# robo-alex/gs-dynamics

Measured on AMD Instinct MI355X. Metric: fwd+bwd Mpix/s at 100k Gaussians, 4x800^2 views, higher is better.
Workload: dtype f32

## Files before the change

### gs-dynamics_amd/csrc/gsr_binning.hip

```cpp
#include "gsr_common.h"

namespace gsr_binning {

#define SCAN_THREADS 1024
#define SCAN_ITEMS 8
__global__ __launch_bounds__(SCAN_THREADS) void scan_exclusive_kernel(const uint32_t* __restrict__ in,
                                                                      uint32_t* __restrict__ out, uint32_t n,
                                                                      uint32_t* __restrict__ total_out) {
  __shared__ uint32_t wave_tot[SCAN_THREADS / GSR_WAVE];
  __shared__ uint32_t carry_s;
  const int tid = threadIdx.x, lane = tid & 63, wv = tid >> 6;
  if (tid == 0) carry_s = 0;
  __syncthreads();
  const uint32_t per_round = SCAN_THREADS * SCAN_ITEMS;
  for (uint32_t base = 0; base < n; base += per_round) {
    uint32_t v[SCAN_ITEMS];
    uint32_t first = base + (uint32_t)tid * SCAN_ITEMS;
    uint32_t sum = 0;
#pragma unroll
    for (int k = 0; k < SCAN_ITEMS; ++k) {
      uint32_t idx = first + k;
      v[k] = idx < n ? in[idx] : 0u;
      sum += v[k];
    }
// ... 616 lines not shown
  const int Ts = gsr_bin_stride(tab.T), rows = tab.rows, t = blockIdx.x * GSR_BLOCK + threadIdx.x;
  if (t >= Ts) return;
  uint32_t* __restrict__ m = vw.tile_rows;
  uint32_t run = 0;
  int r = 0;
  for (; r + 8 <= rows; r += 8) {
    uint32_t v[8];
#pragma unroll
    for (int u = 0; u < 8; ++u) v[u] = m[(size_t)(r + u) * Ts + t];
#pragma unroll
    for (int u = 0; u < 8; ++u) { m[(size_t)(r + u) * Ts + t] = run; run += v[u]; }
  }
  for (; r < rows; ++r) { const uint32_t v = m[(size_t)r * Ts + t]; m[(size_t)r * Ts + t] = run; run += v; }
  m[(size_t)rows * Ts + t] = run;
}

__global__ __launch_bounds__(GSR_BLOCK) void bin_colprefix_scan_kernel(GsrBinViews tab) {
  const GsrBinView& vw = tab.v[blockIdx.y];
  if (vw.shares_lists) return;
  __shared__ uint32_t s_w[GSR_BLOCK / 64];
  __shared__ uint32_t s_base;
  const int T = tab.T, Ts = gsr_bin_stride(T), rows = tab.rows, tid = threadIdx.x, lane = tid & 63, wv = tid >> 6;
  const int t = blockIdx.x * GSR_BLOCK + tid;
  uint32_t* __restrict__ m = vw.tile_rows;
  uint32_t run = 0;
  if (t < Ts) {
    int r = 0;
    for (; r + 8 <= rows; r += 8) {
      uint32_t v[8];
#pragma unroll
      for (int u = 0; u < 8; ++u) v[u] = m[(size_t)(r + u) * Ts + t];
#pragma unroll
      for (int u = 0; u < 8; ++u) { m[(size_t)(r + u) * Ts + t] = run; run += v[u]; }
    }
    for (; r < rows; ++r) { const uint32_t v = m[(size_t)r * Ts + t]; m[(size_t)r * Ts + t] = run; run += v; }
    m[(size_t)rows * Ts + t] = run;
  }
  uint32_t inc = run;
#pragma unroll
  for (int d = 1; d < 64; d <<= 1) {
    const uint32_t o = __shfl_up(inc, d, 64);
    if (lane >= d) inc += o;
  }
  if (lane == 63) s_w[wv] = inc;
  __syncthreads();
  uint32_t before = 0, total = 0;
#pragma unroll
  for (int w = 0; w < GSR_BLOCK / 64; ++w) { if (w < wv) before += s_w[w]; total += s_w[w]; }
  uint32_t* __restrict__ words = vw.block_hist;
  if (tid == 0) __hip_atomic_store(&words[blockIdx.x], 0x80000000u | total, __ATOMIC_RELAXED, __HIP_MEMORY_SCOPE_AGENT);
  if (wv == 0) {
    uint32_t mine = 0;
    if (lane < (int)blockIdx.x) {
      uint32_t w;
      do { w = __hip_atomic_load(&words[lane], __ATOMIC_RELAXED, __HIP_MEMORY_SCOPE_AGENT); } while (!(w & 0x80000000u));
      mine = w & 0x7fffffffu;
    }
#pragma unroll
    for (int k = 32; k >= 1; k >>= 1) mine += __shfl_xor(mine, k, 64);
    if (lane == 0) s_base = mine;
  }
  __syncthreads();
  const uint32_t start = s_base + before + inc - run, cap = vw.D;
  if (t < T) vw.ranges[t] = make_uint2(min(start, cap), min(start + run, cap));
}

__device__ __forceinline__ void bin_scan_view(const GsrBinViews& tab, const GsrBinView& vw, int prefixed, uint32_t* s_wave, uint32_t* s_carry) {
  const int T = tab.T, Ts = gsr_bin_stride(T), rows = tab.rows, tid = threadIdx.x, lane = tid & 63, wv = tid >> 6;
  uint32_t* __restrict__ m = vw.tile_rows;
  const uint32_t cap = vw.D;
  if (tid == 0) *s_carry = 0;
  __syncthreads();
  for (int q0 = 0; q0 < Ts / 4; q0 += BIN_THREADS) {
    const int q = q0 + tid;
    const bool live = q < Ts / 4;
    uint4 tot = make_uint4(0u, 0u, 0u, 0u);
    if (live) {
      if (prefixed) tot = *reinterpret_cast<const uint4*>(m + (size_t)rows * Ts + 4 * q);
      else {
        for (int r0 = 0; r0 < rows; r0 += BIN_ROW_CHUNK) {
          uint4 v[BIN_ROW_CHUNK];
#pragma unroll
          for (int r = 0; r < BIN_ROW_CHUNK; ++r)
            v[r] = r0 + r < rows ? *reinterpret_cast<const uint4*>(m + (size_t)(r0 + r) * Ts + 4 * q) : make_uint4(0u, 0u, 0u, 0u);
#pragma unroll
          for (int r = 0; r < BIN_ROW_CHUNK; ++r)
            if (r0 + r < rows) {
              *reinterpret_cast<uint4*>(m + (size_t)(r0 + r) * Ts + 4 * q) = tot;
              tot.x += v[r].x; tot.y += v[r].y; tot.z += v[r].z; tot.w += v[r].w;
            }
        }
      }
    }
    const uint32_t mine = tot.x + tot.y + tot.z + tot.w;
    uint32_t inc = mine;
#pragma unroll
    for (int d = 1; d < 64; d <<= 1) {
      const uint32_t o = __shfl_up(inc, d, 64);
      if (lane >= d) inc += o;
    }
    if (lane == 63) s_wave[wv] = inc;
    __syncthreads();
    uint32_t start = *s_carry + inc - mine;
    for (int w = 0; w < wv; ++w) start += s_wave[w];
    if (live) {
      const uint32_t c[4] = {tot.x, tot.y, tot.z, tot.w};
      uint32_t st_ = start;
#pragma unroll
      for (int k = 0; k < 4; ++k) {
        if (4 * q + k < T) vw.ranges[4 * q + k] = make_uint2(min(st_, cap), min(st_ + c[k], cap));
        st_ += c[k];
      }
    }
    __syncthreads();
    if (tid == BIN_THREADS - 1) *s_carry = start + mine;
    __syncthreads();
  }
}

__global__ __launch_bounds__(BIN_THREADS) void bin_scan_kernel(GsrBinViews tab, int prefixed) {
  __shared__ uint32_t s_wave[BIN_THREADS / 64];
  __shared__ uint32_t s_carry;
  const GsrBinView& vw = tab.v[blockIdx.x];
  if (vw.shares_lists) return;
  bin_scan_view(tab, vw, prefixed, s_wave, &s_carry);
}

__global__ __launch_bounds__(BIN_THREADS) void bin_emit_kernel(int P, GsrBinViews tab, int order_wgs, int items_per_wg) {
  extern __shared__ uint32_t s_cur[];
  if ((int)blockIdx.x >= tab.rows) {
    __shared__ TileOrderLds L;
    if (blockIdx.y == 0) tile_order_body(tab, items_per_wg, (int)blockIdx.x - tab.rows, L);
    return;
  }
  (void)order_wgs;
  __shared__ uint2 s_big[BIN_BIG_MAX];
  __shared__ uint64_t s_bigkey[BIN_BIG_MAX];
  __shared__ uint32_t s_nbig;
  const GsrBinView& vw = tab.v[blockIdx.y];
  const int T = tab.T, Ts = gsr_bin_stride(T), gx = tab.gx, tid = threadIdx.x, lane = tid & 63, wv = tid >> 6;
  const int g0 = (int)blockIdx.x * GSR_BIN_G;
  if (vw.shares_lists) return;
  const uint32_t cap = vw.D;
  const uint32_t* __restrict__ row = vw.tile_rows + (size_t)blockIdx.x * Ts;
  const uint32_t* __restrict__ cut = vw.depth_cut;
  const bool cut_l = cut && tab.cut_lds;
  const uint32_t* s_cut = s_cur + T;
  const uint32_t* s_cc = s_cur + 2 * T;
  const int gxc = (gx + 3) >> 2;
  if (cut_l)
    for (int t = tid; t < T; t += BIN_THREADS) s_cur[T + t] = cut[t];
  auto cut_at = [&](uint32_t t) { return cut_l ? s_cut[t] : cut[t]; };
  auto behind_all = [&](uint2 r, uint32_t dbits) {
    const uint32_t x0 = (r.x & 0xffffu) >> 2, y0 = (r.x >> 16) >> 2, x1 = ((r.y & 0xffffu) - 1u) >> 2, y1 = ((r.y >> 16) - 1u) >> 2;
    uint32_t m = 0u;
    for (uint32_t y = y0; y <= y1; ++y)
      for (uint32_t x = x0; x <= x1; ++x) m = max(m, s_cc[y * gxc + x]);
    return dbits > m;
  };
  uint64_t* __restrict__ dg = vw.dg[0];
  uint2 rc[BIN_PER_THREAD], ek[BIN_PER_THREAD];
#pragma unroll
  for (int q = 0; q < BIN_PER_THREAD; ++q) {
    const int g = g0 + tid * BIN_PER_THREAD + q;
    rc[q] = make_uint2(0u, 0u); ek[q] = rc[q];
    if (g < P) { rc[q] = vw.rect[g]; ek[q] = vw.ekey[g]; }
  }
  if (tid == 0) s_nbig = 0;
  for (int t = tid; t < T; t += BIN_THREADS) s_cur[t] = vw.ranges[t].x + row[t];
  __syncthreads();
  if (cut_l) {
    const int gyc = (T / gx + 3) >> 2;
    for (int c = tid; c < gxc * gyc; c += BIN_THREADS) {
      const int cx = c % gxc, cy = c / gxc;
      uint32_t m = 0u;
      for (int y = 4 * cy; y < min(4 * cy + 4, T / gx); ++y)
        for (int x = 4 * cx; x < min(4 * cx + 4, gx); ++x) m = max(m, s_cut[y * gx + x]);
      s_cur[2 * T + c] = m;
    }
    __syncthreads();
  }
#pragma unroll
  for (int q = 0; q < BIN_PER_THREAD; ++q) {
    const BinGauss b = bin_gauss(rc[q], ek[q].y);
    if (b.area == 0u) continue;
    if (cut_l && behind_all(rc[q], ek[q].x)) continue;
    const uint64_t key = ((uint64_t)ek[q].x << 32) | (uint32_t)(g0 + tid * BIN_PER_THREAD + q);
    if (b.area > BIN_BIG_AREA) {
      const uint32_t slot = atomicAdd(&s_nbig, 1u);
      if (slot < BIN_BIG_MAX) { s_big[slot] = rc[q]; s_bigkey[slot] = key; continue; }
    }
    const uint32_t dbits = ek[q].x;
    bin_for_tiles(b, gx, [&](uint32_t t) {
      if (cut && dbits > cut_at(t)) return;
      const uint32_t slot = atomicAdd(&s_cur[t], 1u);
      if (slot < cap) dg[slot] = key;
    });
  }
  __syncthreads();
  const uint32_t nbig = min(s_nbig, (uint32_t)BIN_BIG_MAX);
  for (uint32_t i = wv; i < nbig; i += BIN_THREADS / 64) {
    const BinGauss b = bin_gauss(s_big[i], 0u);
    const uint64_t key = s_bigkey[i];
    for (uint32_t k = lane; k < b.area; k += 64) {
      const uint32_t t = bin_tile_of(b, k, gx);
      if (cut && (uint32_t)(key >> 32) > cut_at(t)) continue;
      const uint32_t slot = atomicAdd(&s_cur[t], 1u);
      if (slot < cap) dg[slot] = key;
    }
  }
}

__global__ __launch_bounds__(GSR_BLOCK) void tile_ranges_kernel(GsrBinViews tab, int cur) {
  const GsrBinView& vw = tab.v[blockIdx.y];
  const uint32_t* __restrict__ tkey = vw.tkey[cur];
  uint2* __restrict__ ranges = vw.ranges;
  const uint32_t D = bin_entries(vw);
  uint32_t i = blockIdx.x * GSR_BLOCK + threadIdx.x;
  if (i >= D) return;
  uint32_t t = tkey[i];
  if (i == 0) ranges[t].x = 0;
  else {
    uint32_t pt = tkey[i - 1];
    if (pt != t) { ranges[pt].y = i; ranges[t].x = i; }
  }
  if (i == D - 1) ranges[t].y = D;
}


template <typename PTR>
__device__ __forceinline__ void tile_sort_network(PTR a, uint32_t n, int tid, const uint32_t NT = GSR_BLOCK) {
  uint32_t lg = 1;
  while ((1u << lg) < n) ++lg;
  const uint32_t npairs = (1u << lg) >> 1;
  for (uint32_t lk = 1; lk <= lg; ++lk) {
    const uint32_t k = 1u << lk, hk = k >> 1;
    for (uint32_t p = tid; p < npairs; p += NT) {
      const uint32_t base = (p >> (lk - 1)) << lk, off = p & (hk - 1);
      const uint32_t l = base + off, r = base + (k - 1 - off);
      if (r < n) {
        uint64_t x = a[l], y = a[r];
        if (y < x) { a[l] = y; a[r] = x; }
      }
    }
    __syncthreads();
    for (int lj = (int)lk - 2; lj >= 0; --lj) {
      const uint32_t j = 1u << lj;
      for (uint32_t p = tid; p < npairs; p += NT) {
        const uint32_t l = ((p >> lj) << (lj + 1)) + (p & (j - 1)), r = l + j;
        if (r < n) {
          uint64_t x = a[l], y = a[r];
          if (y < x) { a[l] = y; a[r] = x; }
        }
      }
      __syncthreads();
    }
  }
}

template <int M>
__device__ __forceinline__ uint32_t gsr_lane_xor(uint32_t v) {
  if constexpr (M == 1) return (uint32_t)__builtin_amdgcn_update_dpp(0, (int)v, 0xB1, 0xf, 0xf, true);
  else if constexpr (M == 2) return (uint32_t)__builtin_amdgcn_update_dpp(0, (int)v, 0x4E, 0xf, 0xf, true);
  else if constexpr (M == 3) return (uint32_t)__builtin_amdgcn_update_dpp(0, (int)v, 0x1B, 0xf, 0xf, true);
  else if constexpr (M == 7) return (uint32_t)__builtin_amdgcn_update_dpp(0, (int)v, 0x141, 0xf, 0xf, true);
  else if constexpr (M == 15) return (uint32_t)__builtin_amdgcn_update_dpp(0, (int)v, 0x140, 0xf, 0xf, true);
  else if constexpr (M == 8) return (uint32_t)__builtin_amdgcn_update_dpp(0, (int)v, 0x128, 0xf, 0xf, true);
  else if constexpr (M < 32) return (uint32_t)__builtin_amdgcn_ds_swizzle((int)v, (M << 10) | 0x1F);
  else return (uint32_t)__shfl_xor((int)v, M, 64);
}
template <int V> struct gsr_log2 { static constexpr int value = 1 + gsr_log2<(V >> 1)>::value; };
template <> struct gsr_log2<1> { static constexpr int value = 0; };
template <int MASK, int NR>
__device__ __forceinline__ void wave_sort_step(uint64_t (&x)[NR], int lane) {
  constexpr int LR = gsr_log2<NR>::value;
  constexpr int R = MASK & (NR - 1), L = MASK >> LR;
  constexpr int HB = MASK >= 1024 ? 1024 : MASK >= 512 ? 512 : MASK >= 256 ? 256 : MASK >= 128 ? 128 : MASK >= 64 ? 64 : MASK >= 32 ? 32 : MASK >= 16 ? 16 : MASK >= 8 ? 8 : MASK >= 4 ? 4 : MASK >= 2 ? 2 : 1;
  if constexpr (L == 0) {
#pragma unroll
    for (int r = 0; r < NR; ++r) {
      if ((r & HB) == 0) {
        const uint64_t a = x[r], b = x[r ^ R];
        const bool sw = b < a;
        x[r] = sw ? b : a;
        x[r ^ R] = sw ? a : b;
      }
    }
  } else {
    uint64_t y[NR];
#pragma unroll
    for (int r = 0; r < NR; ++r) {
      const uint64_t src = x[r ^ R];
      y[r] = ((uint64_t)gsr_lane_xor<L>((uint32_t)(src >> 32)) << 32) | gsr_lane_xor<L>((uint32_t)src);
    }
    const bool upper = (lane & (HB >> LR)) != 0;
#pragma unroll
    for (int r = 0; r < NR; ++r) {
      const bool take = (y[r] < x[r]) != upper;
      x[r] = take ? y[r] : x[r];
    }
  }
}
template <int LK, int NR>
__device__ __forceinline__ void wave_sort_stage(uint64_t (&x)[NR], int lane) {
  static_assert(LK <= 11, "the half-cleaner steps below stop at stride 512");
  wave_sort_step<(1 << LK) - 1, NR>(x, lane);
  if constexpr (LK >= 11) wave_sort_step<512, NR>(x, lane);
  if constexpr (LK >= 10) wave_sort_step<256, NR>(x, lane);
  if constexpr (LK >= 9) wave_sort_step<128, NR>(x, lane);
  if constexpr (LK >= 8) wave_sort_step<64, NR>(x, lane);
  if constexpr (LK >= 7) wave_sort_step<32, NR>(x, lane);
  if constexpr (LK >= 6) wave_sort_step<16, NR>(x, lane);
  if constexpr (LK >= 5) wave_sort_step<8, NR>(x, lane);
  if constexpr (LK >= 4) wave_sort_step<4, NR>(x, lane);
  if constexpr (LK >= 3) wave_sort_step<2, NR>(x, lane);
  if constexpr (LK >= 2) wave_sort_step<1, NR>(x, lane);
}
template <int NR>
__device__ __forceinline__ void wave_sort_tile(const uint64_t* __restrict__ seg, uint32_t* __restrict__ out, uint32_t n, int lane) {
  uint64_t x[NR];
#pragma unroll
  for (int r = 0; r < NR; ++r) { const uint32_t e = (uint32_t)(r * 64 + lane); x[r] = e < n ? seg[e] : ~0ull; }
  wave_sort_stage<1, NR>(x, lane); wave_sort_stage<2, NR>(x, lane); wave_sort_stage<3, NR>(x, lane);
  wave_sort_stage<4, NR>(x, lane); wave_sort_stage<5, NR>(x, lane); wave_sort_stage<6, NR>(x, lane);
  if constexpr (NR >= 2) wave_sort_stage<7, NR>(x, lane);
  if constexpr (NR >= 4) wave_sort_stage<8, NR>(x, lane);
  if constexpr (NR >= 8) wave_sort_stage<9, NR>(x, lane);
  if constexpr (NR >= 16) wave_sort_stage<10, NR>(x, lane);
  if constexpr (NR >= 32) wave_sort_stage<11, NR>(x, lane);
  const uint32_t e0 = (uint32_t)lane * NR;
  if constexpr (NR >= 4) {
    if ((((uintptr_t)out) & 15u) == 0 && e0 + NR <= n) {
#pragma unroll
      for (int r = 0; r < NR; r += 4)
        *reinterpret_cast<uint4*>(out + e0 + r) = make_uint4((uint32_t)x[r], (uint32_t)x[r + 1], (uint32_t)x[r + 2], (uint32_t)x[r + 3]);
      return;
    }
  }
#pragma unroll
  for (int r = 0; r < NR; ++r) if (e0 + r < n) out[e0 + r] = (uint32_t)x[r];
}

template <int RCAP, int NW = 4>
struct TileSortLds {
  union {
    struct { uint32_t key[2][RCAP]; uint32_t val[2][RCAP]; } r;
    uint64_t net[2 * RCAP];
  };
  uint32_t whist[NW][256];
  uint32_t wtot[4];
  uint32_t diff;
};

template <int RCAP, int NW>
__device__ __forceinline__ int tile_radix_sort(TileSortLds<RCAP, NW>& L, uint32_t n, int tid) {
  constexpr int NT = 64 * NW;
  const int lane = tid & 63, wv = tid >> 6;
  const uint32_t q = ((n + (uint32_t)NT - 1u) / (uint32_t)NT) << 6;
  const uint32_t wstart = min(n, (uint32_t)wv * q), wstop = min(n, wstart + q);
  const uint32_t diff = L.diff;
  int cur = 0;
  for (int shift = 0; shift < 32; shift += 8) {
    if (((diff >> shift) & 0xffu) == 0u) continue;
    const uint32_t* __restrict__ kin = L.r.key[cur];
    const uint32_t* __restrict__ vin = L.r.val[cur];
    uint32_t* __restrict__ kout = L.r.key[cur ^ 1];
    uint32_t* __restrict__ vout = L.r.val[cur ^ 1];
    for (int i = tid; i < NW * 256; i += NT) (&L.whist[0][0])[i] = 0;
    __syncthreads();
    for (uint32_t i = wstart + lane; i < wstop; i += 64) atomicAdd(&L.whist[wv][(kin[i] >> shift) & 0xffu], 1u);
    __syncthreads();
    {
      uint32_t c[NW], tot = 0;
      if (tid < 256) {
#pragma unroll
        for (int w = 0; w < NW; ++w) { c[w] = L.whist[w][tid]; tot += c[w]; }
      }
      uint32_t inc = tot;
#pragma unroll
      for (int d = 1; d < 64; d <<= 1) {
        const uint32_t o = __shfl_up(inc, d, 64);
        if (lane >= d) inc += o;
      }
      if (tid < 256 && lane == 63) L.wtot[wv] = inc;
      __syncthreads();
      if (tid < 256) {
        uint32_t base = inc - tot;
        for (int w = 0; w < wv; ++w) base += L.wtot[w];
#pragma unroll
        for (int w = 0; w < NW; ++w) { L.whist[w][tid] = base; base += c[w]; }
      }
    }
    __syncthreads();
    volatile uint32_t* wbase = L.whist[wv];
    for (uint32_t i0 = wstart; i0 < wstop; i0 += 64) {
      const uint32_t i = i0 + lane;
      const bool valid = i < wstop;
      uint32_t key = 0, val = 0;
      if (valid) { key = kin[i]; val = vin[i]; }
      const uint32_t digit = (key >> shift) & 0xffu;
      const uint64_t peers = match_peers(digit, valid, 8);
      const uint32_t rank = (uint32_t)__popcll(peers & gsr_lanemask_lt());
      uint32_t pos = 0;
      if (valid) pos = wbase[digit] + rank;
      __builtin_amdgcn_wave_barrier();
      if (valid && rank == 0) wbase[digit] = pos + (uint32_t)__popcll(peers);
      __builtin_amdgcn_wave_barrier();
      if (valid) { kout[pos] = key; vout[pos] = val; }
    }
    __syncthreads();
    cur ^= 1;
  }
  return cur;
}

template <int RCAP, int NW>
__device__ __forceinline__ void tile_sort_long_ticket(const GsrBinViews& tab, int cur, uint32_t ticket);

#ifndef TS_W32_WAVES
#define TS_W32_WAVES 5
#endif
#ifndef TS_MIN_WAVES
#define TS_MIN_WAVES 7
#endif
template <int RCAP, int MODE = 0, int NW = 4>
__global__ __launch_bounds__(64 * NW, (RCAP <= 1024 || MODE == 2) ? TS_MIN_WAVES : (MODE == 3 ? TS_W32_WAVES : 1)) void tile_sort_kernel(GsrBinViews tab, int cur) {
  const int tid = threadIdx.x;
  if constexpr (MODE == 3) {
    const uint32_t n_long3 = tab.queue[6], n_mid = tab.queue[3];
    const uint32_t ticket = n_long3 + blockIdx.x * 4u + (uint32_t)(tid >> 6);
    if (ticket >= n_mid) return;
    const uint4 ord = tab.order[ticket];
    const GsrBinView& vw = tab.v[__builtin_amdgcn_readfirstlane(ord.w)];
    if (vw.shares_lists) return;
    const uint32_t n = __builtin_amdgcn_readfirstlane(ord.z - ord.y);
    wave_sort_tile<32>(vw.dg[cur] + ord.y, vw.point_list + ord.y, n, tid & 63);
    return;
  }
  const uint32_t n_busy = tab.queue[4], n_long = tab.queue[6];
  if (MODE == 2 || (MODE == 0 && blockIdx.x >= n_long)) {
    const uint32_t first = (MODE == 2 && tab.wave_cap == 2048) ? tab.queue[3] : n_long;
    const uint32_t ticket = first + (MODE == 2 ? blockIdx.x : blockIdx.x - n_long) * 4u + (uint32_t)(tid >> 6);
    if (ticket >= n_busy) return;
    const uint4 ord = tab.order[ticket];
    const GsrBinView& vw = tab.v[__builtin_amdgcn_readfirstlane(ord.w)];
    if (vw.shares_lists) return;
    const uint32_t n = __builtin_amdgcn_readfirstlane(ord.z - ord.y);
    const uint64_t* seg = vw.dg[cur] + ord.y;
    uint32_t* out = vw.point_list + ord.y;
    if (n <= 64) wave_sort_tile<1>(seg, out, n, tid & 63);
    else if (n <= 128) wave_sort_tile<2>(seg, out, n, tid & 63);
    else if (n <= 256) wave_sort_tile<4>(seg, out, n, tid & 63);
    else if (n <= 512) wave_sort_tile<8>(seg, out, n, tid & 63);
    else wave_sort_tile<16>(seg, out, n, tid & 63);
    return;
  }
  if constexpr (MODE == 1) {
    const uint32_t n_mine = tab.wave_cap == 512 ? tab.queue[2] : n_long;
    for (uint32_t ticket = blockIdx.x; ticket < n_mine; ticket += gridDim.x) {
      tile_sort_long_ticket<RCAP, NW>(tab, cur, ticket);
      __syncthreads();
    }
  } else if constexpr (MODE != 2) {
    if (blockIdx.x >= n_long) return;
    if (RCAP <= 1024 && tab.vlong_launch && blockIdx.x < tab.queue[2]) return;
    tile_sort_long_ticket<RCAP, NW>(tab, cur, blockIdx.x);
  }
}

template <int RCAP, int NW>
__device__ __forceinline__ void tile_sort_long_ticket(const GsrBinViews& tab, int cur, uint32_t ticket) {
  __shared__ TileSortLds<RCAP, NW> L;
  constexpr uint32_t NT = 64 * NW;
  const int tid = threadIdx.x;
  const uint4 ord = tab.order[ticket];
  const GsrBinView& vw = tab.v[__builtin_amdgcn_readfirstlane(ord.w)];
  if (vw.shares_lists) return;
  uint64_t* __restrict__ dg = vw.dg[cur];
  uint32_t* __restrict__ point_list = vw.point_list;
  const uint2 rg = make_uint2(ord.y, ord.z);
  const uint32_t n = rg.y - rg.x;
  if (n == 0) return;
  uint64_t* seg = dg + rg.x;
  if (n == 1) {
    if (tid == 0) point_list[rg.x] = (uint32_t)seg[0];
  } else if (n <= (uint32_t)RCAP) {
    if (tid == 0) L.diff = 0;
    __syncthreads();
    const uint32_t k0 = (uint32_t)(seg[0] >> 32);
    uint32_t d = 0;
    for (uint32_t i = tid; i < n; i += NT) {
      const uint64_t e = seg[i];
      const uint32_t k = (uint32_t)(e >> 32);
      L.r.key[0][i] = k; L.r.val[0][i] = (uint32_t)e;
      d |= k ^ k0;
    }
    if (d) atomicOr(&L.diff, d);
    __syncthreads();
    const int cur = tile_radix_sort(L, n, tid);
    {
      uint32_t* __restrict__ kk = L.r.key[cur];
      uint32_t* __restrict__ vv = L.r.val[cur];
      bool long_run = false;
      for (uint32_t i = tid; i + 1 < n; i += NT) {
        if (kk[i] == kk[i + 1] && (i == 0 || kk[i - 1] != kk[i])) {
          uint32_t j = i + 1;
          while (j + 1 < n && kk[j + 1] == kk[i] && j - i < 32u) ++j;
          if (j + 1 < n && kk[j + 1] == kk[i]) { long_run = true; continue; }
          for (uint32_t a = i + 1; a <= j; ++a) {
            const uint32_t x = vv[a];
            uint32_t b = a;
            while (b > i && vv[b - 1] > x) { vv[b] = vv[b - 1]; --b; }
            vv[b] = x;
          }
        }
      }
      if (__syncthreads_or(long_run ? 1 : 0)) {
        uint64_t e[(RCAP + NT - 1) / NT];
#pragma unroll
        for (int u = 0; u < (RCAP + NT - 1) / NT; ++u) {
          const uint32_t i = (uint32_t)u * NT + tid;
          e[u] = i < n ? (((uint64_t)kk[i] << 32) | vv[i]) : 0ull;
        }
        __syncthreads();
#pragma unroll
        for (int u = 0; u < (RCAP + NT - 1) / NT; ++u) {
          const uint32_t i = (uint32_t)u * NT + tid;
          if (i < n) L.net[i] = e[u];
        }
        __syncthreads();
        tile_sort_network(L.net, n, tid, NT);
        for (uint32_t i = tid; i < n; i += NT) point_list[rg.x + i] = (uint32_t)L.net[i];
        return;
      }
    }
    for (uint32_t i = tid; i < n; i += NT) point_list[rg.x + i] = L.r.val[cur][i];
  } else if (n <= 2u * (uint32_t)RCAP) {
    for (uint32_t i = tid; i < n; i += NT) L.net[i] = seg[i];
    __syncthreads();
    tile_sort_network(L.net, n, tid, NT);
    for (uint32_t i = tid; i < n; i += NT) point_list[rg.x + i] = (uint32_t)L.net[i];
  } else {
    __syncthreads();
    tile_sort_network((volatile uint64_t*)seg, n, tid, NT);
    for (uint32_t i = tid; i < n; i += NT) point_list[rg.x + i] = (uint32_t)seg[i];
  }
}

__global__ __launch_bounds__(GSR_BLOCK) void copy_tile_state_kernel(int T, int n_order, const uint2* __restrict__ src_ranges,
                                                                    const uint4* __restrict__ src_order, const uint32_t* __restrict__ src_queue,
                                                                    uint2* __restrict__ ranges, uint4* __restrict__ order, uint32_t* __restrict__ queue) {
  const int i = blockIdx.x * GSR_BLOCK + threadIdx.x;
  if (i < T) ranges[i] = src_ranges[i];
  if (i < n_order) order[i] = src_order[i];
  if (i < 9) queue[i] = (i == 4 || i == 6 || i == 7) ? src_queue[i] : 0u;
}

}
using namespace gsr_binning;

int gsr_launch_shared_lists(const GsrBinViews& tab_in, int P, uint32_t D, const uint2* owner_ranges, const uint4* owner_order,
                            const uint32_t* owner_queue, uint2* ranges, uint4* order, uint32_t* queue, hipStream_t st) {
  GsrBinViews tab = tab_in;
  tab.v[0].shares_lists = 1;
  { GSR_PROF("emit_entries", st);
    hipLaunchKernelGGL(emit_entries_kernel, dim3(D / GSR_RADIX_EPB + 1u, 1), dim3(GSR_BLOCK), 0, st, P, tab, 0, 1); }
  GSR_HIP_CHECK(hipGetLastError());
  { GSR_PROF("copy_tile_state", st);
    hipLaunchKernelGGL(copy_tile_state_kernel, dim3((tab.T + GSR_BLOCK - 1) / GSR_BLOCK), dim3(GSR_BLOCK), 0, st, tab.T, tab.T, owner_ranges,
                       owner_order, owner_queue, ranges, order, queue); }
  GSR_HIP_CHECK(hipGetLastError());
  return 0;
}

int gsr_launch_scan_exclusive(const uint32_t* in, uint32_t* out, uint32_t n, uint32_t* total_out, hipStream_t st) {
  { GSR_PROF("scan", st);
  hipLaunchKernelGGL(scan_exclusive_kernel, dim3(1), dim3(SCAN_THREADS), 0, st, in, out, n, total_out); }
  GSR_HIP_CHECK(hipGetLastError());
  return 0;
}

static int ceil_log2_u32(uint32_t n) {
  int b = 0;
  while (((uint64_t)1 << b) < n) ++b;
  return b;
}

static size_t bin_lds_limit() {
  static const size_t v = [] {
    int dev = 0, a = 0;
    if (hipGetDevice(&dev) == hipSuccess && hipDeviceGetAttribute(&a, hipDeviceAttributeMaxSharedMemoryPerBlock, dev) == hipSuccess && a > 0) return (size_t)a;
    return (size_t)(64 << 10);
  }();
  return v;
}
static size_t bin_lds_static() {
  static const size_t v = [] {
    hipFuncAttributes a{}, b{};
    size_t m = 0;
    if (hipFuncGetAttributes(&a, reinterpret_cast<const void*>(bin_emit_kernel)) == hipSuccess) m = a.sharedSizeBytes;
    if (hipFuncGetAttributes(&b, reinterpret_cast<const void*>(bin_count_kernel)) == hipSuccess && b.sharedSizeBytes > m) m = b.sharedSizeBytes;
    return m ? m : (size_t)(52 << 10);
  }();
  return v;
}
bool gsr_rows_path_ok(int T) {
  const char* e = getenv("GSR_RADIX_BINNING");
  const bool radix_only = e && *e && atoi(e) != 0;
  return !radix_only && T > 0 && T <= GSR_BIN_MAX_T && bin_lds_static() + sizeof(uint32_t) * (size_t)T <= bin_lds_limit();
}
int gsr_launch_binning(const GsrBinViews& tab_in, int P, hipStream_t st) {
  if (tab_in.V <= 0 || tab_in.T <= 0) return 0;
  GsrBinViews tab = tab_in;
  uint32_t maxD = 0, maxblk = 0;
  for (int v = 0; v < tab.V; ++v) { maxD = tab.v[v].D > maxD ? tab.v[v].D : maxD; maxblk = tab.v[v].nblocks > maxblk ? tab.v[v].nblocks : maxblk; }
  const char* force = getenv("GSR_TILE_SORT_RCAP");
  const bool big = force ? (force[0] == '4') : (maxD / (uint32_t)tab.T > 600u);
  tab.wave_cap = big ? 2048 : 512;
  {
    static uint32_t* hint = [] { uint32_t* p = nullptr; if (hipHostMalloc((void**)&p, 64, hipHostMallocMapped | hipHostMallocCoherent) != hipSuccess) return (uint32_t*)nullptr; *p = 1u; return p; }();
    tab.vlong_out = hint;
    tab.vlong_launch = (!hint || __atomic_load_n(hint, __ATOMIC_RELAXED) != 0u) ? 1 : 0;
  }
  int cur = 0;
  bool order_done = false;
  bool any_cut = false;
  for (int v = 0; v < tab.V; ++v) any_cut = any_cut || tab.v[v].depth_cut != nullptr;
  const size_t coarse = (size_t)((tab.gx + 3) / 4) * (size_t)((tab.T / tab.gx + 3) / 4);
  tab.cut_lds = (any_cut && bin_lds_static() + sizeof(uint32_t) * (2 * (size_t)tab.T + coarse) <= bin_lds_limit()) ? 1 : 0;
  const size_t lds = sizeof(uint32_t) * (tab.cut_lds ? 2 * (size_t)tab.T + coarse : (size_t)tab.T);
  const bool rows_path = tab.rows > 0 && gsr_rows_path_ok(tab.T) && maxD > 0 && P > 0;
  if (rows_path) {
    { GSR_PROF("bin_count", st);
      hipLaunchKernelGGL(bin_count_kernel, dim3(tab.rows, tab.V), dim3(BIN_THREADS), lds, st, P, tab);
    }
    GSR_HIP_CHECK(hipGetLastError());
    const int prefixed = tab.rows > BIN_DIRECT_ROWS ? 1 : 0;
    const int col_wgs = (gsr_bin_stride(tab.T) + GSR_BLOCK - 1) / GSR_BLOCK;
    const bool chained = prefixed && col_wgs <= 64;
    if (chained) {
      GSR_PROF("bin_colprefix", st);
      hipLaunchKernelGGL(bin_colprefix_scan_kernel, dim3(col_wgs, tab.V), dim3(GSR_BLOCK), 0, st, tab);
    } else if (prefixed) {
      GSR_PROF("bin_colprefix", st);
      hipLaunchKernelGGL(bin_colprefix_kernel, dim3(col_wgs, tab.V), dim3(GSR_BLOCK), 0, st, tab);
    }
    GSR_HIP_CHECK(hipGetLastError());
    const int n_items = tab.V * ((tab.T + 1023) / 1024);
    if (!chained) {
      GSR_PROF("bin_scan", st);
      hipLaunchKernelGGL(bin_scan_kernel, dim3(tab.V), dim3(BIN_THREADS), 0, st, tab, prefixed);
    }
    GSR_HIP_CHECK(hipGetLastError());
    int order_wgs = 0, per_wg = 1;
    {
      order_wgs = n_items < ORD_MAX_WG ? n_items : ORD_MAX_WG;
      if (order_wgs < 1) order_wgs = 1;
      per_wg = (n_items + order_wgs - 1) / order_wgs;
      if (per_wg < 1) per_wg = 1;
      order_wgs = (n_items + per_wg - 1) / per_wg;
      if (order_wgs < 1) order_wgs = 1;
      order_done = true;
    }
    { GSR_PROF("bin_emit", st);
      hipLaunchKernelGGL(bin_emit_kernel, dim3(tab.rows + order_wgs, tab.V), dim3(BIN_THREADS), lds, st, P, tab, order_wgs, per_wg); }
    GSR_HIP_CHECK(hipGetLastError());
  } else if (maxD == 0 || P <= 0) {
    for (int v = 0; v < tab.V; ++v) GSR_HIP_CHECK(hipMemsetAsync(tab.v[v].ranges, 0, sizeof(uint2) * (size_t)tab.T, st));
  } else {
    const int tbits = ceil_log2_u32((uint32_t)tab.T);
    const int npass = (tbits + 7) / 8;
    const int bpp = npass ? (tbits + npass - 1) / npass : 0;
    { GSR_PROF("emit_entries", st);
    const int bits0 = npass ? (tbits < bpp ? tbits : bpp) : 1;
    hipLaunchKernelGGL(emit_entries_kernel, dim3(maxD / GSR_RADIX_EPB + 1u, tab.V), dim3(GSR_BLOCK), 0, st, P, tab, 0, bits0); }
    GSR_HIP_CHECK(hipGetLastError());
    for (int pass = 0; pass < npass; ++pass) {
      const int shift = pass * bpp;
      const int bits = (tbits - shift) < bpp ? (tbits - shift) : bpp;
      if (pass > 0) {
        GSR_PROF("radix_hist", st);
        hipLaunchKernelGGL(radix_hist_kernel, dim3(maxblk, tab.V), dim3(GSR_BLOCK), 0, st, tab, cur, shift, bits);
      }
      GSR_HIP_CHECK(hipGetLastError());
      const int prescanned = maxblk >= GSR_COLSCAN_MIN_BLOCKS ? 1 : 0;
      if (prescanned) {
        GSR_PROF("radix_colscan", st);
        hipLaunchKernelGGL(radix_colscan_kernel, dim3(1u << bits, tab.V), dim3(1024), 0, st, tab, bits);
      }
      GSR_HIP_CHECK(hipGetLastError());
      { GSR_PROF("radix_scatter", st);
      hipLaunchKernelGGL(radix_scatter_kernel, dim3(maxblk, tab.V), dim3(GSR_BLOCK), 0, st, tab, cur, shift, bits, prescanned,
                         pass == npass - 1 ? 1 : 0); }
      GSR_HIP_CHECK(hipGetLastError());
      cur ^= 1;
    }
    if (npass == 0) {
      GSR_PROF("tile_ranges", st);
      hipLaunchKernelGGL(tile_ranges_kernel, dim3((maxD + GSR_BLOCK - 1) / GSR_BLOCK, tab.V), dim3(GSR_BLOCK), 0, st, tab, cur);
    }
    GSR_HIP_CHECK(hipGetLastError());
  }
  if (!order_done)
    if (int rc = gsr_launch_tile_order(tab, st)) return rc;
  if (maxD > 0 && P > 0) {
    { GSR_PROF("tile_sort", st);
    if (big) {
      hipLaunchKernelGGL((tile_sort_kernel<2048, 2>), dim3((tab.V * tab.T + 3) / 4), dim3(GSR_BLOCK), 0, st, tab, cur);
      if (tab.wave_cap == 2048) hipLaunchKernelGGL((tile_sort_kernel<2048, 3>), dim3((tab.V * tab.T + 3) / 4), dim3(GSR_BLOCK), 0, st, tab, cur);
      const int g1 = tab.V * tab.T < 512 ? tab.V * tab.T : 512;
      hipLaunchKernelGGL((tile_sort_kernel<4096, 1, 8>), dim3(g1), dim3(512), 0, st, tab, cur);
    } else
      {
        const bool small_lds = !(force && force[0] == '2');
        if (small_lds) {
          hipLaunchKernelGGL(tile_sort_kernel<1024>, dim3(tab.V * tab.T), dim3(GSR_BLOCK), 0, st, tab, cur);
          if (tab.vlong_launch) hipLaunchKernelGGL((tile_sort_kernel<4096, 1, 16>), dim3(64), dim3(1024), 0, st, tab, cur);
        } else hipLaunchKernelGGL(tile_sort_kernel<2048>, dim3(tab.V * tab.T), dim3(GSR_BLOCK), 0, st, tab, cur);
      } }
    GSR_HIP_CHECK(hipGetLastError());
  }
  return 0;
}

int gsr_launch_tile_order(const GsrBinViews& tab, hipStream_t st) {
  { GSR_PROF("tile_order", st);
    const int n_items = tab.V * ((tab.T + 1023) / 1024);
    int wgs = n_items < ORD_MAX_WG ? n_items : ORD_MAX_WG;
    if (wgs < 1) wgs = 1;
    const int per_wg = (n_items + wgs - 1) / wgs;
    wgs = per_wg > 0 ? (n_items + per_wg - 1) / per_wg : 1;
    hipLaunchKernelGGL(tile_order_kernel, dim3(wgs < 1 ? 1 : wgs), dim3(1024), 0, st, tab, per_wg > 0 ? per_wg : 1); }
  GSR_HIP_CHECK(hipGetLastError());
  return 0;
}
```

Baseline: 5581.

## Sort long tiles with paired-wave bitonic merge through LDS instead of block radix sort

For long tiles (beyond 512 keys, when wave_cap is 512), two waves now each sort one half of the tile in registers with a bitonic network. They exchange halves through shared memory and finish with a merge and half-cleaner stages. Each 4-wave block handles two such tickets, replacing the block-wide multi-pass radix sort per long tile, and the wave-sort block indexing is shifted to make room. It also adds optional, compile-time-disabled timing trace instrumentation. The cost is more LDS traffic and added code complexity.

Measured after the change: 5725 (median of 6 runs). 2.6% higher.

```diff
diff --git a/gs-dynamics_amd/csrc/gsr_binning.hip b/gs-dynamics_amd/csrc/gsr_binning.hip
--- a/gs-dynamics_amd/csrc/gsr_binning.hip
+++ b/gs-dynamics_amd/csrc/gsr_binning.hip
@@ -942,9 +942,15 @@
   }
 }
 template <int LK, int NR>
+__device__ __forceinline__ void wave_sort_halfcleaners(uint64_t (&x)[NR], int lane);
+template <int LK, int NR>
 __device__ __forceinline__ void wave_sort_stage(uint64_t (&x)[NR], int lane) {
+  wave_sort_step<(1 << LK) - 1, NR>(x, lane);
+  wave_sort_halfcleaners<LK, NR>(x, lane);
+}
+template <int LK, int NR>
+__device__ __forceinline__ void wave_sort_halfcleaners(uint64_t (&x)[NR], int lane) {
   static_assert(LK <= 11, "the half-cleaner steps below stop at stride 512");
-  wave_sort_step<(1 << LK) - 1, NR>(x, lane);
   if constexpr (LK >= 11) wave_sort_step<512, NR>(x, lane);
   if constexpr (LK >= 10) wave_sort_step<256, NR>(x, lane);
   if constexpr (LK >= 9) wave_sort_step<128, NR>(x, lane);
@@ -957,6 +963,8 @@
   if constexpr (LK >= 2) wave_sort_step<1, NR>(x, lane);
 }
 template <int NR>
+__device__ __forceinline__ void wave_sort_store(const uint64_t (&x)[NR], uint32_t* __restrict__ out, uint32_t e0, uint32_t n);
+template <int NR>
 __device__ __forceinline__ void wave_sort_tile(const uint64_t* __restrict__ seg, uint32_t* __restrict__ out, uint32_t n, int lane) {
   uint64_t x[NR];
 #pragma unroll
@@ -968,7 +976,10 @@
   if constexpr (NR >= 8) wave_sort_stage<9, NR>(x, lane);
   if constexpr (NR >= 16) wave_sort_stage<10, NR>(x, lane);
   if constexpr (NR >= 32) wave_sort_stage<11, NR>(x, lane);
-  const uint32_t e0 = (uint32_t)lane * NR;
+  wave_sort_store<NR>(x, out, (uint32_t)lane * NR, n);
+}
+template <int NR>
+__device__ __forceinline__ void wave_sort_store(const uint64_t (&x)[NR], uint32_t* __restrict__ out, uint32_t e0, uint32_t n) {
   if constexpr (NR >= 4) {
     if ((((uintptr_t)out) & 15u) == 0 && e0 + NR <= n) {
 #pragma unroll
@@ -1055,6 +1066,91 @@
 }
 
 template <int RCAP, int NW>
+__device__ __forceinline__ TileSortLds<RCAP, NW>& tile_sort_lds() {
+  __shared__ TileSortLds<RCAP, NW> L;
+  return L;
+}
+__device__ __forceinline__ uint32_t pair_slot(uint32_t pos, uint32_t lnr) { return ((pos & ((1u << lnr) - 1u)) << 6) + (pos >> lnr); }
+template <int NR>
+__device__ __forceinline__ void pair_upper_sort(uint64_t (&x)[8], uint64_t* __restrict__ mine, const uint64_t* __restrict__ seg, uint32_t n, int lane) {
+  constexpr int LNR = gsr_log2<NR>::value;
+  uint64_t y[NR];
+#pragma unroll
+  for (int r = 0; r < NR; ++r) { const uint32_t e = 512u + (uint32_t)(r * 64 + lane); y[r] = e < n ? seg[e] : ~0ull; }
+  wave_sort_stage<1, NR>(y, lane); wave_sort_stage<2, NR>(y, lane); wave_sort_stage<3, NR>(y, lane);
+  wave_sort_stage<4, NR>(y, lane); wave_sort_stage<5, NR>(y, lane); wave_sort_stage<6, NR>(y, lane);
+  if constexpr (NR >= 2) wave_sort_stage<7, NR>(y, lane);
+  if constexpr (NR >= 4) wave_sort_stage<8, NR>(y, lane);
+  if constexpr (NR >= 8) wave_sort_stage<9, NR>(y, lane);
+#pragma unroll
+  for (int r = 0; r < NR; ++r) { mine[pair_slot((uint32_t)(lane * NR + r), LNR)] = y[r]; x[r] = y[r]; }
+}
+template <int NR>
+__device__ __forceinline__ void pair_upper_merge(uint64_t (&x)[8], const uint64_t* __restrict__ lower, uint32_t* __restrict__ out, uint32_t n, int lane) {
+  uint64_t y[NR];
+#pragma unroll
+  for (int r = 0; r < NR; ++r) {
+    const uint64_t o = lower[pair_slot(511u - (uint32_t)(lane * NR + r), 3)];
+    y[r] = o > x[r] ? o : x[r];
+  }
+  wave_sort_halfcleaners<gsr_log2<NR>::value + 7, NR>(y, lane);
+  wave_sort_store<NR>(y, out, 512u + (uint32_t)lane * NR, n);
+}
+template <int RCAP, int NW>
+__device__ __forceinline__ void tile_sort_pair_tickets(const GsrBinViews& tab, int cur, uint32_t ticket0, uint32_t n_long) {
+  static_assert(NW == 4 && 2 * RCAP >= 4 * 512, "two pairs of waves, 512 keys per wave in the network block");
+  TileSortLds<RCAP, NW>& L = tile_sort_lds<RCAP, NW>();
+  const int tid = threadIdx.x, lane = tid & 63, wv = tid >> 6;
+  const bool upper = (wv & 1) != 0;
+  const uint32_t ticket = ticket0 + (uint32_t)(wv >> 1);
+  bool live = ticket < n_long;
+  uint32_t n = 0;
+  const uint64_t* seg = nullptr;
+  uint32_t* out = nullptr;
+  if (live) {
+    const uint4 ord = tab.order[ticket];
+    const GsrBinView& vw = tab.v[__builtin_amdgcn_readfirstlane(ord.w)];
+    live = !vw.shares_lists;
+    n = __builtin_amdgcn_readfirstlane(ord.z - ord.y);
+    seg = vw.dg[cur] + ord.y;
+    out = vw.point_list + ord.y;
+  }
+  const uint32_t m = n > 512u ? n - 512u : 0u;
+  const uint32_t lnru = m <= 64u ? 0u : m <= 128u ? 1u : m <= 256u ? 2u : 3u;
+  uint64_t x[8];
+  uint64_t* mine = L.net + wv * 512;
+  if (live && !upper) {
+#pragma unroll
+    for (int r = 0; r < 8; ++r) { const uint32_t e = (uint32_t)(r * 64 + lane); x[r] = e < n ? seg[e] : ~0ull; }
+    wave_sort_stage<1, 8>(x, lane); wave_sort_stage<2, 8>(x, lane); wave_sort_stage<3, 8>(x, lane);
+    wave_sort_stage<4, 8>(x, lane); wave_sort_stage<5, 8>(x, lane); wave_sort_stage<6, 8>(x, lane);
+    wave_sort_stage<7, 8>(x, lane); wave_sort_stage<8, 8>(x, lane); wave_sort_stage<9, 8>(x, lane);
+#pragma unroll
+    for (int r = 0; r < 8; ++r) mine[pair_slot((uint32_t)(lane * 8 + r), 3)] = x[r];
+  } else if (live) {
+    if (lnru == 0u) pair_upper_sort<1>(x, mine, seg, n, lane);
+    else if (lnru == 1u) pair_upper_sort<2>(x, mine, seg, n, lane);
+    else if (lnru == 2u) pair_upper_sort<4>(x, mine, seg, n, lane);
+    else pair_upper_sort<8>(x, mine, seg, n, lane);
+  }
+  __syncthreads();
+  if (!live) return;
+  const uint64_t* theirs = L.net + (wv ^ 1) * 512;
+  if (!upper) {
+#pragma unroll
+    for (int r = 0; r < 8; ++r) {
+      const uint32_t j = 511u - (uint32_t)(lane * 8 + r);
+      if (j < (64u << lnru)) { const uint64_t o = theirs[pair_slot(j, lnru)]; x[r] = o < x[r] ? o : x[r]; }
+    }
+    wave_sort_halfcleaners<10, 8>(x, lane);
+    wave_sort_store<8>(x, out, (uint32_t)lane * 8u, n);
+  } else if (lnru == 0u) pair_upper_merge<1>(x, theirs, out, n, lane);
+  else if (lnru == 1u) pair_upper_merge<2>(x, theirs, out, n, lane);
+  else if (lnru == 2u) pair_upper_merge<4>(x, theirs, out, n, lane);
+  else pair_upper_merge<8>(x, theirs, out, n, lane);
+}
+
+template <int RCAP, int NW>
 __device__ __forceinline__ void tile_sort_long_ticket(const GsrBinViews& tab, int cur, uint32_t ticket);
 
 #ifndef TS_W32_WAVES
@@ -1063,9 +1159,23 @@
 #ifndef TS_MIN_WAVES
 #define TS_MIN_WAVES 7
 #endif
+#ifdef GSR_TRACE_SORT
+#define GSR_SORT_TRACE_MAX 65536
+__device__ uint4 g_sort_trace[GSR_SORT_TRACE_MAX];
+__device__ uint32_t g_sort_wg_start[GSR_SORT_TRACE_MAX];
+#define GSR_SORT_TRACE(ticket, kind, n)                                                                     \
+  do { if ((threadIdx.x & ((kind) == 2 ? 127 : 63)) == 0 && ((kind) != 1 || threadIdx.x == 0) && (ticket) < GSR_SORT_TRACE_MAX) \
+         g_sort_trace[ticket] = make_uint4((uint32_t)tr0, (uint32_t)wall_clock64(), blockIdx.x | ((uint32_t)(kind) << 24), n); } while (0)
+#else
+#define GSR_SORT_TRACE(ticket, kind, n) do { } while (0)
+#endif
 template <int RCAP, int MODE = 0, int NW = 4>
 __global__ __launch_bounds__(64 * NW, (RCAP <= 1024 || MODE == 2) ? TS_MIN_WAVES : (MODE == 3 ? TS_W32_WAVES : 1)) void tile_sort_kernel(GsrBinViews tab, int cur) {
   const int tid = threadIdx.x;
+#ifdef GSR_TRACE_SORT
+  unsigned long long tr0 = wall_clock64();
+  if (MODE == 0 && tid == 0 && blockIdx.x < GSR_SORT_TRACE_MAX) g_sort_wg_start[blockIdx.x] = (uint32_t)tr0;
+#endif
   if constexpr (MODE == 3) {
     const uint32_t n_long3 = tab.queue[6], n_mid = tab.queue[3];
     const uint32_t ticket = n_long3 + blockIdx.x * 4u + (uint32_t)(tid >> 6);
@@ -1075,12 +1185,29 @@
     if (vw.shares_lists) return;
     const uint32_t n = __builtin_amdgcn_readfirstlane(ord.z - ord.y);
     wave_sort_tile<32>(vw.dg[cur] + ord.y, vw.point_list + ord.y, n, tid & 63);
+    GSR_SORT_TRACE(ticket, 3, n);
     return;
   }
   const uint32_t n_busy = tab.queue[4], n_long = tab.queue[6];
-  if (MODE == 2 || (MODE == 0 && blockIdx.x >= n_long)) {
+  uint32_t wave_block0 = n_long;
+  if constexpr (MODE == 0 && RCAP <= 1024) {
+    if (tab.wave_cap == 512) {
+      const uint32_t n_vlong = min(tab.queue[2], n_long);
+      wave_block0 = n_vlong + ((n_long - n_vlong + 1u) >> 1);
+      if (blockIdx.x >= n_vlong && blockIdx.x < wave_block0) {
+        const uint32_t ticket0 = n_vlong + 2u * (blockIdx.x - n_vlong);
+        tile_sort_pair_tickets<RCAP, NW>(tab, cur, ticket0, n_long);
+#ifdef GSR_TRACE_SORT
+        const uint32_t tk = ticket0 + (uint32_t)(tid >> 7);
+        if (tk < n_long) GSR_SORT_TRACE(tk, 2, tab.order[tk].z - tab.order[tk].y);
+#endif
+        return;
+      }
+    }
+  }
+  if (MODE == 2 || (MODE == 0 && blockIdx.x >= wave_block0)) {
     const uint32_t first = (MODE == 2 && tab.wave_cap == 2048) ? tab.queue[3] : n_long;
-    const uint32_t ticket = first + (MODE == 2 ? blockIdx.x : blockIdx.x - n_long) * 4u + (uint32_t)(tid >> 6);
+    const uint32_t ticket = first + (MODE == 2 ? blockIdx.x : blockIdx.x - wave_block0) * 4u + (uint32_t)(tid >> 6);
     if (ticket >= n_busy) return;
     const uint4 ord = tab.order[ticket];
     const GsrBinView& vw = tab.v[__builtin_amdgcn_readfirstlane(ord.w)];
@@ -1093,24 +1220,30 @@
     else if (n <= 256) wave_sort_tile<4>(seg, out, n, tid & 63);
     else if (n <= 512) wave_sort_tile<8>(seg, out, n, tid & 63);
     else wave_sort_tile<16>(seg, out, n, tid & 63);
+    GSR_SORT_TRACE(ticket, 0, n);
     return;
   }
   if constexpr (MODE == 1) {
     const uint32_t n_mine = tab.wave_cap == 512 ? tab.queue[2] : n_long;
     for (uint32_t ticket = blockIdx.x; ticket < n_mine; ticket += gridDim.x) {
       tile_sort_long_ticket<RCAP, NW>(tab, cur, ticket);
+      GSR_SORT_TRACE(ticket, 1, tab.order[ticket].z - tab.order[ticket].y);
       __syncthreads();
+#ifdef GSR_TRACE_SORT
+      tr0 = wall_clock64();
+#endif
     }
   } else if constexpr (MODE != 2) {
     if (blockIdx.x >= n_long) return;
     if (RCAP <= 1024 && tab.vlong_launch && blockIdx.x < tab.queue[2]) return;
     tile_sort_long_ticket<RCAP, NW>(tab, cur, blockIdx.x);
+    GSR_SORT_TRACE(blockIdx.x, 1, tab.order[blockIdx.x].z - tab.order[blockIdx.x].y);
   }
 }
 
 template <int RCAP, int NW>
 __device__ __forceinline__ void tile_sort_long_ticket(const GsrBinViews& tab, int cur, uint32_t ticket) {
-  __shared__ TileSortLds<RCAP, NW> L;
+  TileSortLds<RCAP, NW>& L = tile_sort_lds<RCAP, NW>();
   constexpr uint32_t NT = 64 * NW;
   const int tid = threadIdx.x;
   const uint4 ord = tab.order[ticket];
@@ -1212,6 +1345,16 @@
   GSR_HIP_CHECK(hipGetLastError());
   return 0;
 }
+
+#ifdef GSR_TRACE_SORT
+extern "C" int gsr_debug_sort_trace(uint32_t* out4, uint32_t* wg_start, int n) {
+  GSR_HIP_CHECK(hipDeviceSynchronize());
+  const size_t m = (size_t)(n < GSR_SORT_TRACE_MAX ? n : GSR_SORT_TRACE_MAX);
+  GSR_HIP_CHECK(hipMemcpyFromSymbol(out4, HIP_SYMBOL(g_sort_trace), sizeof(uint4) * m));
+  GSR_HIP_CHECK(hipMemcpyFromSymbol(wg_start, HIP_SYMBOL(g_sort_wg_start), sizeof(uint32_t) * m));
+  return 0;
+}
+#endif
 
 int gsr_launch_scan_exclusive(const uint32_t* in, uint32_t* out, uint32_t n, uint32_t* total_out, hipStream_t st) {
   { GSR_PROF("scan", st);
```
